# peterrum/deal-and-ceed-on-gpu

Measured on AMD Instinct MI355X. Metric: BP5 DoFs/sec per CG iter (p=4, ~1e8 DoFs) + % HBM roofline at 1/2/4/8 GPUs, higher is better.
Workload: dtype f64

## Files before the change

### deal-and-ceed-on-gpu_amd/_lib.py

```python
import ctypes as C
import os
import re
import subprocess

import numpy as np

_HERE = os.path.dirname(os.path.abspath(__file__))
_ROOT = os.path.dirname(_HERE)
_LIB = None

QUAD_GAUSS, QUAD_GLL, QUAD_GAUSS_OVER = 0, 1, 2
COEF_ONE, COEF_STEP64 = 0, 1
CG_PLAIN, CG_MERGED = 0, 1
GEOM_MERGED6, GEOM_AFFINE, GEOM_TRILINEAR = 0, 1, 2
OP_POISSON, OP_HELMHOLTZ, OP_MASS = 0, 1, 2
UNIQUE_ID_BYTES = 128
MAX_COMPONENTS = 8


class BP5Error(RuntimeError):
    def __init__(self, status, detail):
        super().__init__(f"bp5 status {status}: {detail}")
        self.status = status

# ... 123 lines not shown
        "bp5_mf_compute_merged_metric": (i32, [vp, vp]),
        "bp5_mf_metric_to_reference_layout": (i32, [vp, vp, vp]),
        "bp5_mf_set_geometry_mode": (i32, [vp, i32]),
        "bp5_mf_get_data": (i32, [vp, i32, C.POINTER(MFData)]),
        "bp5_apply": (i32, [vp, vp, vp, vp, i32]),
        "bp5_apply_cells": (i32, [vp, vp, vp, vp, u32, u32]),
        "bp5_apply_components": (i32, [vp, vp, i32, sz, vp, vp, i32]),
        "bp5_copy_constrained": (i32, [vp, vp, vp]),
        "bp5_set_constrained": (i32, [vp, f64, vp]),
        "bp5_mf_set_apply_variant": (i32, [vp, i32]),
        "bp5_mf_get_apply_variant": (i32, [vp, C.POINTER(C.c_int)]),
        "bp5_mf_set_block_workgroups": (i32, [vp, i32]),
        "bp5_mf_set_streaming": (i32, [vp, i32]),
        "bp5_mf_set_tuning": (i32, [vp, i32, i32]),
        "bp5_mf_get_tuning": (i32, [vp, i32, C.POINTER(C.c_int)]),
        "bp5_mf_wait_value_available": (i32, [vp, C.POINTER(C.c_int)]),
        "bp5_mf_block_plan_info": (i32, [vp, C.POINTER(C.c_uint32), C.POINTER(C.c_uint32), C.POINTER(C.c_int)]),
        "bp5_assemble_rhs": (i32, [vp, vp]),
        "bp5_compute_diagonal": (i32, [vp, vp, vp, i32]),
        "bp5_l2_norm_solution": (i32, [vp, vp, C.POINTER(f64)]),
        "bp5_vec_fill": (i32, [vp, vp, f64, sz]),
        "bp5_vec_axpy": (i32, [vp, vp, f64, vp, sz]),
        "bp5_vec_equ": (i32, [vp, vp, f64, vp, sz]),
        "bp5_vec_sadd": (i32, [vp, vp, f64, f64, vp, sz]),
        "bp5_vec_dot": (i32, [vp, vp, vp, sz, C.POINTER(f64)]),
        "bp5_vec_l2_norm": (i32, [vp, vp, C.c_size_t, C.POINTER(C.c_double)]),
        "bp5_vec_all_zero": (i32, [vp, vp, C.c_size_t, C.POINTER(C.c_int)]),
        "bp5_comm_unique_id": (i32, [vp]),
        "bp5_comm_create": (i32, [vp, i32, i32, C.POINTER(vp)]),
        "bp5_comm_destroy": (i32, [vp]),
# ... 105 lines not shown
```

### deal-and-ceed-on-gpu_amd/csrc/bp5_device.hip

```cpp
#include "bp5_device.hpp"


extern "C" int bp5_device_count(int *count)
{
  if (!count) return fail(BP5_ERR_INVALID, "null argument");
  int c = 0;
  hipError_t e = hipGetDeviceCount(&c);
  if (e != hipSuccess) { *count = 0; return fail(BP5_ERR_NO_DEVICE, hipGetErrorString(e)); }
  *count = c;
  return BP5_OK;
}
extern "C" int bp5_vec_alloc(size_t n, double **out)
{
  if (!out) return fail(BP5_ERR_INVALID, "null argument");
  HIP_TRY(hipMalloc((void **)out, std::max<size_t>(n, 1) * sizeof(double)));
  HIP_TRY(hipMemset(*out, 0, std::max<size_t>(n, 1) * sizeof(double)));
  HIP_TRY(hipStreamSynchronize(nullptr));
  return BP5_OK;
}
extern "C" int bp5_vec_free(double *v) { HIP_TRY(hipFree(v)); return BP5_OK; }
extern "C" int bp5_copy_h2d(void *dst, const void *src, size_t bytes) { HIP_TRY(hipMemcpy(dst, src, bytes, hipMemcpyHostToDevice)); return BP5_OK; }
extern "C" int bp5_copy_d2h(void *dst, const void *src, size_t bytes) { HIP_TRY(hipMemcpy(dst, src, bytes, hipMemcpyDeviceToHost)); return BP5_OK; }

static void tuning_from_environment(bp5_mf *mf);
// ... 139 lines not shown
  HIP_TRY(hipHostMalloc((void **)&mf->h_st, ST_COUNT * sizeof(int)));
  HIP_TRY(hipEventCreate(&mf->ev_solve[0]));
  HIP_TRY(hipEventCreate(&mf->ev_solve[1]));
  guard.m = nullptr;
  *out = mf;
  return BP5_OK;
}

extern "C" int bp5_mf_destroy(bp5_mf *mf)
{
  if (!mf) return BP5_OK;
  hipSetDevice(mf->device);
  hipStreamSynchronize(mf->stream);
  void *ptrs[] = {mf->d_constrained_bits, mf->d_l2g, mf->d_constrained, mf->d_send_idx, mf->d_coords, mf->d_tab, mf->d_tab_gauss, mf->d_l2g_padded,
                  mf->d_constraint_mask, mf->d_inv_jac, mf->d_JxW, mf->d_qpoints, mf->d_sendbuf, mf->d_recvbuf, mf->d_partials,
                  mf->d_sc, mf->d_scalar, mf->d_st, mf->ws_base, mf->d_stamps, mf->d_evec, mf->d_scalar_plane, mf->d_gcell, mf->d_vertices, mf->d_hang_mask, mf->d_hang_I, mf->d_send_dirichlet, mf->d_signal, mf->ws_z, mf->wsc_base, mf->wsz_base, mf->wsn_base, mf->hc_base, mf->d_hc_off};
  for (void *p : ptrs) if (p) hipFree(p);
  if (mf->h_sc) hipHostFree(mf->h_sc);
  if (mf->h_st) hipHostFree(mf->h_st);
  for (hipEvent_t e : mf->ev_pool) hipEventDestroy(e);
  for (hipEvent_t e : mf->phase.ev) hipEventDestroy(e);
  for (hipEvent_t e : mf->ev_solve) if (e) hipEventDestroy(e);
  for (hipEvent_t e : mf->ev_halo) if (e) hipEventDestroy(e);
  for (hipEvent_t e : mf->ev_done) if (e) hipEventDestroy(e);
  if (mf->h_done) hipHostFree(mf->h_done);
  if (mf->comm_stream) { hipStreamSynchronize(mf->comm_stream); hipStreamDestroy(mf->comm_stream); }
  for (auto &kv : mf->march_plans) { hipFree(kv.second.team_off); hipFree(kv.second.entries); }
  for (auto &kv : mf->plans) {
    auto &q = kv.second;
    void *pp[] = {q.off, q.dofs, q.sh_dof, q.sh_off, q.sh_slot, q.pos, q.cell_round, q.team_rounds, q.partial, q.cell_off, q.pass_cell, q.pass_off, q.run_off, q.runs, q.gidx, q.packed, q.lattice, q.cell_pos, q.cr_start, q.cr_dof0, q.cr_soff, q.cr_slots, q.cr_tile};
    for (void *x : pp) if (x) hipFree(x);
// ... 833 lines not shown
      const uint32_t grid = combine_grid(mf, owned_tiles, fuse->n_cols);
      if (ct.n_shared >= (8u << 20)) hipLaunchKernelGGL((combine_runs_kernel<false, true, true>), dim3(grid + cr.ghost_blocks), dim3(256), 0, stream, cr, dp->partial, dst);
      else hipLaunchKernelGGL((combine_runs_kernel<false, true, false>), dim3(grid + cr.ghost_blocks), dim3(256), 0, stream, cr, dp->partial, dst);
      KERNEL_CHECK();
      fuse->n_cols += grid;
      mf->signal_target += cr.ghost_blocks;
      return BP5_OK;
    }
    if (tile1 <= cr.tile0) return BP5_OK;
    const dim3 cgt(tile1 - cr.tile0);
    if (fuse && window != COMBINE_GHOST) {
      cr.cg_p = fuse->p; cr.cg_r = fuse->r; cr.dot_partials = mf->d_partials; cr.dot_col0 = fuse->n_cols;
      cr.n_owned = mf->n_owned; cr.n_tiles = cgt.x; cr.cg_state = mf->d_st;
      if (fuse->n_cols + 1024u + 8u > (uint32_t)PARTIAL_STRIDE) return fail(BP5_ERR_UNSUPPORTED, "no partial-sum columns left for the combine pass");
      const uint32_t grid = combine_grid(mf, cgt.x, fuse->n_cols);
      if (ct.n_shared >= (8u << 20)) hipLaunchKernelGGL((combine_runs_kernel<false, true, true>), dim3(grid), dim3(256), 0, stream, cr, dp->partial, dst);
      else hipLaunchKernelGGL((combine_runs_kernel<false, true, false>), dim3(grid), dim3(256), 0, stream, cr, dp->partial, dst);
      KERNEL_CHECK();
      fuse->n_cols += grid;
      return BP5_OK;
    }
    const bool pairs = ct.n_shared >= (8u << 20) && window != COMBINE_GHOST;
    if (set && pairs) hipLaunchKernelGGL((combine_runs_kernel<false, false, true>), cgt, dim3(256), 0, stream, cr, dp->partial, dst);
    else if (set) hipLaunchKernelGGL((combine_runs_kernel<false, false, false>), cgt, dim3(256), 0, stream, cr, dp->partial, dst);
    else if (pairs) hipLaunchKernelGGL((combine_runs_kernel<true, false, true>), cgt, dim3(256), 0, stream, cr, dp->partial, dst);
    else hipLaunchKernelGGL((combine_runs_kernel<true, false, false>), cgt, dim3(256), 0, stream, cr, dp->partial, dst);
    KERNEL_CHECK();
    return BP5_OK;
  }
  if (set) hipLaunchKernelGGL(combine_kernel<false>, cg, dim3(256), 0, stream, dp->sh_dof, dp->sh_off, dp->sh_slot, dp->partial, dst, dp->n_shared);
  else hipLaunchKernelGGL(combine_kernel<true>, cg, dim3(256), 0, stream, dp->sh_dof, dp->sh_off, dp->sh_slot, dp->partial, dst, dp->n_shared);
  KERNEL_CHECK();
  return BP5_OK;
}
// ... 546 lines not shown
static void tuning_from_environment(bp5_mf *mf)
{
  mf->tune[BP5_TUNE_LATTICE_INDICES] = env_int("BP5_LATTICE_INDICES", 1) != 0;
  mf->tune[BP5_TUNE_EARLY_GATHER] = env_int("BP5_EARLY_GATHER", 1) != 0;
  mf->tune[BP5_TUNE_COMBINE_SIGNAL] = env_int("BP5_COMBINE_SIGNAL", 0) == 1;
  { const char *e = getenv("BP5_BOUNDARY_FIRST"); mf->tune[BP5_TUNE_BOUNDARY_FIRST] = !(e && !strcmp(e, "launches")); }
  mf->tune[BP5_TUNE_FOLD_SMALL] = env_int("BP5_FOLD_SMALL", 1) != 0;
  { const int u = env_int("BP5_UPDATE_UNROLL", 1); mf->tune[BP5_TUNE_UPDATE_UNROLL] = (u == 2 || u == 4) ? u : 1; }
  mf->tune[BP5_TUNE_UPDATE_FLAT] = env_int("BP5_UPDATE_FLAT", 1) != 0;
  { const int v = env_int("BP5_UPDATE_NT", -1); mf->tune[BP5_TUNE_UPDATE_NT] = v < 0 ? -1 : v != 0; }
  { const int v = env_int("BP5_COMBINE_WG_PER_CU", 16); mf->tune[BP5_TUNE_COMBINE_WG_PER_CU] = (v >= 0 && v <= 32) ? v : 16; }
  mf->tune[BP5_TUNE_INTERIOR_STORES] = env_int("BP5_INTERIOR_STORES", 1) != 0;
  mf->tune[BP5_TUNE_GHOST_COMBINE_ON_COMM] = env_int("BP5_GHOST_COMBINE_ON_COMM", 0) != 0;
  mf->tune[BP5_TUNE_FACE_CARRY] = env_int("BP5_FACE_CARRY", 1) != 0;
  { const int v = env_int("BP5_FUSED_UPDATE", -1); mf->tune[BP5_TUNE_FUSED_UPDATE] = (v >= -1 && v <= 1) ? v : -1; }
}
extern "C" int bp5_mf_set_tuning(bp5_mf *mf, int knob, int value)
{
  if (!mf || knob < 0 || knob >= BP5_TUNE_COUNT) return fail(BP5_ERR_INVALID, "unknown tuning knob");
  switch (knob) {
    case BP5_TUNE_UPDATE_UNROLL:
      if (value != 1 && value != 2 && value != 4) return fail(BP5_ERR_INVALID, "BP5_TUNE_UPDATE_UNROLL: 1, 2 or 4");
      break;
    case BP5_TUNE_UPDATE_NT:
      if (value < -1 || value > 1) return fail(BP5_ERR_INVALID, "BP5_TUNE_UPDATE_NT: -1, 0 or 1");
      break;
    case BP5_TUNE_FUSED_UPDATE:
      if (value < -1 || value > 1) return fail(BP5_ERR_INVALID, "BP5_TUNE_FUSED_UPDATE: -1, 0 or 1");
      break;
    case BP5_TUNE_COMBINE_WG_PER_CU:
// ... 460 lines not shown
    while ((size_t)used + 4 > mf->ev_pool.size()) { hipEvent_t e; HIP_TRY(hipEventCreate(&e)); mf->ev_pool.push_back(e); }
    HIP_TRY(hipEventRecord(mf->ev_pool[used + k], mf->stream));
    return BP5_OK;
  }
};

struct SolveState {
  ApplyProfile prof;
  int exchange = EXCHANGE_NONE;
  bool two_parts = false;
  bool gather_in_flight = false;
  bool dst_prezeroed = false, copies_dirichlet = false;
  int upd_mode = 0;
  double *upd_x = nullptr;
  const double *upd_diag = nullptr;
  bool phase_on = false;
  int phase_it = 0;
  uint8_t phase_recorded[bp5_mf::PhaseProfile::MAX_ITERS] = {};
};

static int phase_mark(bp5_mf *mf, SolveState &ss, int k)
{
  if (!ss.phase_on || ss.phase_it >= bp5_mf::PhaseProfile::MAX_ITERS) return BP5_OK;
  HIP_TRY(hipEventRecord(mf->phase.ev[(size_t)ss.phase_it * bp5_mf::PhaseProfile::MARKS + k], mf->stream));
  ss.phase_recorded[ss.phase_it] |= (uint8_t)(1u << k);
  return BP5_OK;
}

static int fused_unsplit(bp5_mf *mf, SolveState &ss, ApplyCall &call, const double *coef, const double *src, double *dst)
{
// ... 117 lines not shown
    BP5_TRY(prof.mark(3));
    if (prof.on) prof.used += 4;
    BP5_TRY(bp5_halo_zero_ghosts(mf, src));
    return bp5_copy_constrained(mf, src, dst);
  }
  const bool owner_scatter = variant_overwrites(mf, effective_variant(mf, 0, mf->n_cells));
  BP5_TRY(prof.mark(0));
  if (zero && !owner_scatter) {
    if (!ss.dst_prezeroed) HIP_TRY(hipMemsetAsync(dst, 0, mf->n_local() * sizeof(double), mf->stream));
    zero = false;
    call.dst_known_zero = true;
  }
  BP5_TRY(prof.mark(1));
  if (prof.on) call.mark_event = mf->ev_pool[prof.used + 2];
  FuseState fuse;
  if (fusing) { fuse.p = src; fuse.r = fuse_r; fuse.upd_mode = ss.upd_mode; fuse.upd_x = ss.upd_x; fuse.upd_diag = ss.upd_diag; call.fuse = &fuse; }
  call.overwrite = zero;
  BP5_TRY(launch_apply(mf, call, coef, src, dst));
  if (fusing) *n_cols = fuse.n_cols;
  if (!call.mark_recorded) BP5_TRY(prof.mark(2));
  BP5_TRY(prof.mark(3));
  if (prof.on) prof.used += 4;
  if (fusing) return BP5_OK;
  if (ss.copies_dirichlet) return BP5_OK;
  return bp5_copy_constrained(mf, src, dst);
}

static int poll_state(bp5_mf *mf)
{
  HIP_TRY(hipMemcpyAsync(mf->h_st, mf->d_st, ST_COUNT * sizeof(int), hipMemcpyDeviceToHost, mf->stream));
  HIP_TRY(hipMemcpyAsync(mf->h_sc, mf->d_sc, SC_COUNT * sizeof(double), hipMemcpyDeviceToHost, mf->stream));
  HIP_TRY(hipStreamSynchronize(mf->stream));
  return BP5_OK;
}

static int solve_begin(bp5_mf *mf, const bp5_cg_params *prm, const ApplyProfile &prof)
{
  hipStream_t s = mf->stream;
  if (prof.on) {
    const size_t want = 4 * (size_t)std::min(prm->max_iter, ApplyProfile::MAX_PROFILED);
// ... 278 lines not shown
#undef BP5_UPR
  };
  const bool early_gather_enabled = mf->tune[BP5_TUNE_EARLY_GATHER] != 0;
  const bool early_gather = fused && dist_solve && early_gather_enabled;
  auto gather_under_update = [&](int mode) -> int {
    BP5_TRY(halo_streams(mf));
    const uint32_t ns = mf->send_off.back();
    if (ns) {
      const dim3 gr((ns + 255) / 256), bl(256);
      if (mode == 0) hipLaunchKernelGGL(cgm_pack_updated_kernel<0>, gr, bl, 0, s, mf->d_send_idx, ns, d, g, h, diag, mf->d_sc, mf->d_st, mf->d_sendbuf);
      else hipLaunchKernelGGL(cgm_pack_updated_kernel<1>, gr, bl, 0, s, mf->d_send_idx, ns, d, g, h, diag, mf->d_sc, mf->d_st, mf->d_sendbuf);
      KERNEL_CHECK();
    }
    return gather_exchange(mf, d, true);
  };
  int it = 1;
  for (; it <= prm->max_iter; ++it) {
    const int mode = it == 1 ? 0 : it % 2 == 0 ? 1 : 2;
    BP5_TRY(phase_mark(mf, ss, 0));
    if (early_gather) { BP5_TRY(gather_under_update(mode)); ss.gather_in_flight = true; }
    if (mode != 0) {
      if (n_first) launch_update_rest(mode); else launch_update(mode);
    }
    ss.upd_mode = n_first ? mode : 0; ss.upd_x = x; ss.upd_diag = diag;
    KERNEL_CHECK();
    BP5_TRY(phase_mark(mf, ss, 1));
    const bool one_launch = fused && !mf->comm;
    if (fused) {
      uint32_t n_cols = 0;
      BP5_TRY(vmult(d, h, g, &n_cols));
      BP5_TRY(phase_mark(mf, ss, 4));
      if (one_launch) hipLaunchKernelGGL(cgm_finalize4_kernel<true>, dim3(1), dim3(FIN4_THREADS), 0, s, mf->d_partials, (int)n_cols, mf->d_sc, mf->d_st);
      else hipLaunchKernelGGL(cgm_finalize4_kernel<false>, dim3(1), dim3(FIN4_THREADS), 0, s, mf->d_partials, (int)n_cols, mf->d_sc, mf->d_st);
    } else {
      BP5_TRY(vmult(d, h, nullptr, nullptr));
      BP5_TRY(phase_mark(mf, ss, 4));
      hipLaunchKernelGGL(cgm_dots_kernel, dim3(grid2), dim3(VB), 0, s, d, g, h, diag, n, mf->d_st, mf->d_partials,
                         fold_small ? (const uint32_t *)mf->d_constrained_bits : (const uint32_t *)nullptr);
      hipLaunchKernelGGL(finalize_kernel<7>, dim3(7), dim3(VB), 0, s, mf->d_partials, grid2, mf->d_sc + SC_R0, mf->d_st);
    }
    KERNEL_CHECK();
    BP5_TRY(phase_mark(mf, ss, 5));
    if (!one_launch) {
      BP5_TRY(bp5_comm_allreduce_sum(mf, mf->d_sc + SC_R0, 7));
      BP5_TRY(phase_mark(mf, ss, 6));
      hipLaunchKernelGGL(cgm_control_kernel, dim3(1), dim3(1), 0, s, mf->d_sc, mf->d_st);
      KERNEL_CHECK();
// ... 1038 lines not shown
```

### deal-and-ceed-on-gpu_amd/csrc/bp5_device.hpp

```cpp
#pragma once
#include "bp5_internal.hpp"
#include "bp5_kernels.hpp"

#include <hip/hip_runtime.h>
#include <rccl/rccl.h>

#include <algorithm>
#include <cmath>
#include <cstdio>
#include <cstdlib>
#include <cstring>
#include <map>
#include <memory>
#include <tuple>
#include <vector>

using namespace bp5;

#define HIP_TRY(expr)                                                                                              \
  do {                                                                                                             \
    hipError_t e_ = (expr);                                                                                        \
    if (e_ != hipSuccess)                                                                                          \
      return fail(e_ == hipErrorNoDevice || e_ == hipErrorInvalidDevice ? BP5_ERR_NO_DEVICE : BP5_ERR_HIP,         \
                  std::string(#expr) + ": " + hipGetErrorString(e_));                                              \
// ... 53 lines not shown
  uint32_t pad = 0;
  std::vector<int> neighbors;
  std::vector<uint32_t> send_off, recv_off;
  double *d_sendbuf = nullptr, *d_recvbuf = nullptr;
  uint8_t *d_send_dirichlet = nullptr;
  bp5_comm *comm = nullptr;
  hipStream_t comm_stream = nullptr;
  hipEvent_t ev_halo[4] = {nullptr, nullptr, nullptr, nullptr};
  int overlap = 2;
  bool overlap_now = false;
  bool cg_fusion = true;
  unsigned long long *d_signal = nullptr;
  uint64_t signal_target = 0;
  int wait_value_ok = -1;
  int can_wait_value = -1;
  int tune[BP5_TUNE_COUNT] = {1, 1, 0, 1, 1, 1, 1, -1, 16, 1, 0, 1, -1};
  bool cell_interiors_first = false;
  double *d_partials = nullptr, *d_sc = nullptr, *d_scalar = nullptr;
  int *d_st = nullptr;
  double *ws_g = nullptr, *ws_d = nullptr, *ws_h = nullptr, *d_evec = nullptr;
  char *ws_base = nullptr;
  double *ws_z = nullptr;
  double *wsc_base = nullptr;
  size_t wsc_cap = 0;
  double *wsz_base = nullptr;
  size_t wsz_cap = 0;
  double *wsn_base = nullptr;
  size_t wsn_cap = 0;
  double *hc_base = nullptr;
  size_t hc_cap = 0;
  uint32_t *d_hc_off = nullptr;
// ... 37 lines not shown
  std::vector<uint32_t> h_block_off;
  struct DevMarch { uint32_t *team_off = nullptr, *entries = nullptr; uint32_t n_teams = 0; };
  std::map<int, DevMarch> march_plans;
  std::map<int, DevPlan> plans;
  size_t n_local() const { return (size_t)n_owned + n_ghost; }
  bool has_neighbors() const { return comm && !neighbors.empty(); }
};

struct FuseState {
  const double *p = nullptr, *r = nullptr;
  uint32_t n_cols = 0;
  bool ghosts_zeroed = false;
  int upd_mode = 0;
  double *upd_x = nullptr;
  const double *upd_diag = nullptr;
};
enum VariantFamily { VARIANT_PENCIL, VARIANT_TEAM, VARIANT_MARCH, VARIANT_BLOCK, VARIANT_BLOCK_SIBLING, VARIANT_HANGING_PENCIL, VARIANT_OTHER };
struct VariantInfo {
  VariantFamily family;
  bool atomic_scatter;
  bool shared_by_atomics;
  bool csr_combine;
  bool overwrites;
};
constexpr VariantInfo decode_variant(int v)
{
  const int b = v % 100;
  const VariantFamily f = b <= 6 ? VARIANT_PENCIL : b >= 10 && b <= 14 ? VARIANT_TEAM : b == 56 ? VARIANT_BLOCK : b >= 48 && b <= 63 ? VARIANT_BLOCK_SIBLING
                        : b >= 70 && b <= 72 ? VARIANT_MARCH : b == 90 ? VARIANT_HANGING_PENCIL : VARIANT_OTHER;
  return {f, v >= 100, b == 54 || b == 55, b == 48, v < 100 && (f == VARIANT_TEAM || f == VARIANT_BLOCK || f == VARIANT_BLOCK_SIBLING)};
// ... 829 lines not shown
```

### deal-and-ceed-on-gpu_amd/csrc/bp5_kernels.hpp

```cpp
#pragma once
#include <hip/hip_runtime.h>
#include <stdint.h>
#include <type_traits>

namespace bp5 {

template <int n>
struct ShapeArg {
  double N[n * n];
  double D[n * n];
};

enum : int {
  BLK_AFFINE = 1024, BLK_SINGLE = 2048, BLK_STAMPS = 4096, BLK_SEQ = 8192, BLK_RUNS = 16384, BLK_NTM = 32768, BLK_UPD = 131072, BLK_PACK = 262144,
  BLK_STAGE = 524288, BLK_FUSE = 1048576, BLK_HANG = 2097152, BLK_LDSADD = 4194304, BLK_HELM = 8388608, BLK_LATT = 16777216,
  BLK_ROLL = 67108864, BLK_CARRY = 268435456,
  BLK_F32M = 536870912,
  BLK_MASS = 1073741824,
  BLK_DEFAULT = BLK_SINGLE | BLK_SEQ | BLK_RUNS | BLK_PACK
};
enum : int {
  PEN_INTERIOR_STORES = 32,
  PEN_NT_LOADS = 256,
  PEN_FULL_OCCUPANCY = 512
// ... 3494 lines not shown
  for (uint32_t j = b + 1; j < e; ++j) s += partial[sh_slot[j]];
  const uint32_t g = sh_dof[i];
  if (ADD) dst[g] += s; else dst[g] = s;
}

struct CombineRuns {
  const uint32_t *start, *dof0, *soff, *slots, *tile_run;
  uint32_t n_shared;
  uint32_t tile0, dof_lo, dof_hi;
  const double *cg_p, *cg_r;
  double *dot_partials;
  uint32_t dot_col0, n_owned, n_tiles;
  const int *cg_state;
  uint32_t ghost_blocks, ghost_tile0;
  unsigned long long *signal;
};
constexpr int COMBINE_TILE = 512;
template <bool ADD, bool DOTS = false, bool PAIR = true>
__global__ void __launch_bounds__(256) combine_runs_kernel(CombineRuns cr, const double *partial, double *dst)
{
  __shared__ uint32_t s_start[COMBINE_TILE + 2], s_dof0[COMBINE_TILE + 1], s_soff[COMBINE_TILE + 2];
  __shared__ double s_red[4][4];
  double ds[4] = {0.0, 0.0, 0.0, 0.0};
  const bool ghost_job = DOTS && blockIdx.x < cr.ghost_blocks;
  const uint32_t bid = blockIdx.x - (DOTS ? cr.ghost_blocks : 0u), nblk = gridDim.x - (DOTS ? cr.ghost_blocks : 0u);
  auto ghost_rows_done = [&](bool stores_pending) {
    if (stores_pending) __syncthreads();
    if (threadIdx.x == 0) {
      if (stores_pending) __builtin_amdgcn_fence(__ATOMIC_RELEASE, "agent");
      __hip_atomic_fetch_add(cr.signal, 1ull, __ATOMIC_RELAXED, __HIP_MEMORY_SCOPE_AGENT);
    }
  };
  if constexpr (DOTS) {
    if (cr.cg_state[0]) {
      if (ghost_job) ghost_rows_done(false);
      return;
    }
  }
  const uint32_t dof_lo = ghost_job ? cr.n_owned : cr.dof_lo, dof_hi = ghost_job ? 0xffffffffu : cr.dof_hi;
  auto finish = [&](uint32_t g, bool dirichlet, double s) {
    if (g < dof_lo || g >= dof_hi) return;
    if (ghost_job) { dst[g] = s; return; }
    if constexpr (DOTS) {
      double vi = s;
      if (dirichlet) {
        vi = cr.cg_p[g];
        if (g < cr.n_owned) ds[0] += vi * (vi - s);
      }
      dst[g] = vi;
      if (g < cr.n_owned) {
// ... 183 lines not shown
    }
  }
  if constexpr (DOTS) {
    if (ghost_job) { ghost_rows_done(true); return; }
    const int lane = threadIdx.x & 63, wave = threadIdx.x >> 6;
#pragma unroll
    for (int k = 0; k < 4; ++k) {
      double v = ds[k];
#pragma unroll
      for (int off = 32; off > 0; off >>= 1) v += __shfl_down(v, off, 64);
      if (lane == 0) s_red[k][wave] = v;
    }
    __syncthreads();
    if (threadIdx.x < 7) {
      const int t = threadIdx.x, k = t < 4 ? t : (t == 4 ? 2 : t == 5 ? 1 : 3);
      cr.dot_partials[t * PARTIAL_STRIDE + cr.dot_col0 + bid] = (s_red[k][0] + s_red[k][1]) + (s_red[k][2] + s_red[k][3]);
    }
  }
}

static __global__ void __launch_bounds__(256) zero_indexed_kernel(const uint32_t *idx, uint32_t n, double *dst)
{
  const uint32_t i = blockIdx.x * 256u + threadIdx.x;
  if (i < n) dst[idx[i]] = 0.0;
}

static __global__ void copy_constrained_kernel(const uint32_t *cdofs, uint32_t n, const double *src, double *dst)
{
  const uint32_t i = blockIdx.x * blockDim.x + threadIdx.x;
  if (i < n) { const uint32_t c = cdofs[i]; dst[c] = src[c]; }
}
// ... 384 lines not shown
template <int MODE, int U = 2, bool ZV = false, bool NTX = false>
__global__ void __launch_bounds__(VB) cgm_update_kernel(double *p, double *r, typename std::conditional<ZV, double, const double>::type *v, double *x,
                                                       const double *diag, size_t n, const double *sc, const int *st)
{
  const bool done = st[ST_DONE];
  if (done && !st[ST_PENDING]) return;
  cgm_update_body<MODE, U, ZV, NTX>(p, r, v, x, diag, n, sc, st, done);
}
template <int MODE, int U, bool NTX>
__global__ void __launch_bounds__(VB) cgm_update_rest_kernel(double *p, double *r, const double *v, double *x, const double *diag, size_t first, size_t n,
                                                            const double *sc, const int *st)
{
  if (st[ST_DONE]) return;
  cgm_update_body<MODE, U, false, NTX>(p + first, r + first, v + first, x + first, diag ? diag + first : nullptr, n, sc, st, false);
}
#ifndef BP5_UPD_UNROLL
#define BP5_UPD_UNROLL 3
#endif
template <int MODE>
__device__ __forceinline__ void block_update_run(const BlockPlan &bp, uint32_t lo, uint32_t hi, int t)
{
  static_assert(MODE == 1 || MODE == 2, "the first iteration's p comes from cgm_init_kernel");
  constexpr int U = BP5_UPD_UNROLL;
  constexpr uint32_t TRIP = 2u * 256u;
  const double *sc = bp.upd_sc;
  const double alpha = sc[SC_ALPHA], beta = sc[SC_BETA];
  const double aob = MODE == 2 ? sc[SC_ALPHA_OLD] / sc[SC_BETA_OLD] : 0.0;
  double *const p = bp.upd_p, *const r = bp.upd_r, *const x = bp.upd_x;
  const double *const v = bp.upd_v, *const diag = bp.upd_diag;
  for (uint32_t base = lo + 2u * (uint32_t)t; base < hi; base += TRIP * U) {
    bp5_d2u pv[U], rv[U], vv[U], xv[U];
#pragma unroll
    for (int u = 0; u < U; ++u) {
      const uint32_t i = base + (uint32_t)u * TRIP;
      pv[u] = rv[u] = vv[u] = xv[u] = bp5_d2u{0.0, 0.0};
      if (i + 1 < hi) {
        pv[u] = __builtin_nontemporal_load(reinterpret_cast<const bp5_d2u *>(p + i));
        rv[u] = __builtin_nontemporal_load(reinterpret_cast<const bp5_d2u *>(r + i));
        vv[u] = __builtin_nontemporal_load(reinterpret_cast<const bp5_d2u *>(v + i));
        if (MODE == 2) xv[u] = __builtin_nontemporal_load(reinterpret_cast<const bp5_d2u *>(x + i));
      } else if (i < hi) {
        pv[u].x = __builtin_nontemporal_load(p + i); rv[u].x = __builtin_nontemporal_load(r + i); vv[u].x = __builtin_nontemporal_load(v + i);
        if (MODE == 2) xv[u].x = __builtin_nontemporal_load(x + i);
      }
    }
#pragma unroll
    for (int u = 0; u < U; ++u) {
      const uint32_t i = base + (uint32_t)u * TRIP;
      if (i >= hi) continue;
      const bool pair = i + 1 < hi;
      double p0 = pv[u].x, p1 = pv[u].y, r0 = rv[u].x, r1 = rv[u].y, x0 = xv[u].x, x1 = xv[u].y;
      cgm_update_one<MODE>(p0, r0, vv[u].x, x0, diag ? diag[i] : 1.0, false, false, alpha, beta, aob);
      if (pair) {
        cgm_update_one<MODE>(p1, r1, vv[u].y, x1, diag ? diag[i + 1] : 1.0, false, false, alpha, beta, aob);
        *reinterpret_cast<bp5_d2u *>(p + i) = bp5_d2u{p0, p1};
        *reinterpret_cast<bp5_d2u *>(r + i) = bp5_d2u{r0, r1};
        if (MODE == 2) __builtin_nontemporal_store(bp5_d2u{x0, x1}, reinterpret_cast<bp5_d2u *>(x + i));
      } else {
        p[i] = p0; r[i] = r0;
        if (MODE == 2) __builtin_nontemporal_store(x0, x + i);
      }
    }
  }
}
template <int MODE>
__global__ void __launch_bounds__(256) cgm_pack_updated_kernel(const uint32_t *idx, uint32_t n, const double *p, const double *r, const double *v,
                                                             const double *diag, const double *sc, const int *st, double *buf)
{
  const uint32_t i = blockIdx.x * 256u + threadIdx.x;
  if (i >= n) return;
  const uint32_t g = idx[i];
  double pi = p[g];
  if (!st[ST_DONE]) {
    double ri = r[g], xi = 0.0;
    const double vi = MODE != 0 ? v[g] : 0.0;
    cgm_update_one<MODE>(pi, ri, vi, xi, diag ? diag[g] : 1.0, false, false, sc[SC_ALPHA], sc[SC_BETA], 0.0);
  }
  buf[i] = pi;
// ... 69 lines not shown
  if (lane == 0) red[wave] = s;
  __syncthreads();
  double *out = sc + SC_R0;
  if (threadIdx.x < 4) {
    const int r = threadIdx.x;
    const double t = (red[4 * r] + red[4 * r + 1]) + (red[4 * r + 2] + red[4 * r + 3]);
    out[r] = t;
    if (r == 1) out[5] = t;
    if (r == 2) out[4] = t;
    if (r == 3) out[6] = t;
  }
  if constexpr (CONTROL) {
    __syncthreads();
    if (threadIdx.x == 0) cgm_control_step(sc, st);
  }
}

static __global__ void cgm_control_kernel(double *sc, int *st) { cgm_control_step(sc, st); }

static __global__ void __launch_bounds__(VB) cgm_init_kernel(const double *b, double *x, double *r, double *p, double *v, const double *diag, size_t n,
                                                     double *partials, bool zero_v)
{
  double acc[2] = {0.0, 0.0};
  const size_t stride = (size_t)gridDim.x * VB;
  for (size_t i = (size_t)blockIdx.x * VB + threadIdx.x; i < n; i += stride) {
    const double ri = -b[i], di = diag ? diag[i] : 1.0;
    x[i] = 0.0; r[i] = ri; p[i] = -(di * ri);
    if (zero_v) v[i] = 0.0;
    acc[0] += ri * ri;
  }
// ... 1119 lines not shown
```

### deal-and-ceed-on-gpu_amd/matrix_free.py

```python
import ctypes as C

import numpy as np

from . import _lib
from ._lib import BP5Error, CG_MERGED, CG_PLAIN, COEF_ONE, QUAD_GAUSS


def _torch():
    import torch
    return torch


def _ptr(t, n_min=0):
    torch = _torch()
    if t is None:
        return None
    if not (isinstance(t, torch.Tensor) and t.is_cuda and t.dtype == torch.float64 and t.is_contiguous()):
        raise BP5Error(1, "expected a contiguous float64 CUDA tensor")
    if t.numel() < n_min:
        raise BP5Error(1, f"vector has {t.numel()} entries, need {n_min}")
    return C.c_void_p(t.data_ptr())


class Communicator:
# ... 120 lines not shown
            raise BP5Error(1, f"metric precision must be 'float64' or 'float32', not {precision!r}")
        _lib.check(_lib.lib().bp5_mf_set_metric_precision(self.handle, self.METRIC_PRECISION[precision]))

    def get_metric_precision(self):
        v = C.c_int()
        _lib.check(_lib.lib().bp5_mf_get_metric_precision(self.handle, C.byref(v)))
        return "float32" if v.value == 1 else "float64"

    def set_block_workgroups(self, n):
        _lib.check(_lib.lib().bp5_mf_set_block_workgroups(self.handle, int(n)))

    def set_streaming(self, policy):
        _lib.check(_lib.lib().bp5_mf_set_streaming(self.handle, int(policy)))

    TUNE = {"lattice_indices": 0, "early_gather": 1, "combine_signal": 2, "boundary_first": 3, "fold_small": 4, "update_unroll": 5,
            "update_flat": 6, "update_nt": 7, "combine_wg_per_cu": 8, "interior_stores": 9, "ghost_combine_on_comm": 10, "face_carry": 11, "fused_update": 12}

    def set_tuning(self, knob, value):
        _lib.check(_lib.lib().bp5_mf_set_tuning(self.handle, int(self.TUNE.get(knob, knob)), int(value)))

    def get_tuning(self, knob):
        v = C.c_int()
        _lib.check(_lib.lib().bp5_mf_get_tuning(self.handle, int(self.TUNE.get(knob, knob)), C.byref(v)))
        return v.value

    def wait_value_available(self):
        v = C.c_int()
        _lib.check(_lib.lib().bp5_mf_wait_value_available(self.handle, C.byref(v)))
        return bool(v.value)

    def block_plan_info(self):
        nb, mr, pk = C.c_uint32(), C.c_uint32(), C.c_int()
        _lib.check(_lib.lib().bp5_mf_block_plan_info(self.handle, C.byref(nb), C.byref(mr), C.byref(pk)))
        return nb.value, mr.value, bool(pk.value)

    def block_plan_lattice(self):
        n = C.c_uint32()
        _lib.check(_lib.lib().bp5_mf_block_plan_lattice(self.handle, C.byref(n)))
        return n.value
# ... 955 lines not shown
```

### include/bp5.h

```cpp
#ifndef BP5_H
#define BP5_H

#include <stddef.h>
#include <stdint.h>

#ifdef __cplusplus
extern "C" {
#endif

enum {
  BP5_OK = 0,
  BP5_ERR_INVALID = 1,
  BP5_ERR_HIP = 2,
  BP5_ERR_NO_DEVICE = 3,
  BP5_ERR_RCCL = 4,
  BP5_ERR_UNSUPPORTED = 5,
  BP5_ERR_BREAKDOWN = 6,
  BP5_ERR_NO_CONVERGENCE = 7
};
const char *bp5_strerror(int status);
const char *bp5_last_error(void);

enum { BP5_QUAD_GAUSS = 0,
       BP5_QUAD_GLL = 1,
// ... 113 lines not shown
int bp5_apply(bp5_mf *mf, const double *coef, const double *src, double *dst, int zero_dst);
int bp5_apply_cells(bp5_mf *mf, const double *coef, const double *src, double *dst, uint32_t cell_begin,
                    uint32_t cell_end);
int bp5_copy_constrained(bp5_mf *mf, const double *src, double *dst);
int bp5_set_constrained(bp5_mf *mf, double value, double *dst);

#define BP5_MAX_COMPONENTS 8
int bp5_apply_components(bp5_mf *mf, const double *coef, int n_components, size_t ld, const double *src, double *dst, int zero_dst);

int bp5_mf_set_apply_variant(bp5_mf *mf, int variant);
int bp5_mf_set_block_workgroups(bp5_mf *mf, int max_workgroups);
int bp5_mf_set_streaming(bp5_mf *mf, int policy);
enum { BP5_TUNE_LATTICE_INDICES = 0, BP5_TUNE_EARLY_GATHER = 1, BP5_TUNE_COMBINE_SIGNAL = 2, BP5_TUNE_BOUNDARY_FIRST = 3,
       BP5_TUNE_FOLD_SMALL = 4, BP5_TUNE_UPDATE_UNROLL = 5, BP5_TUNE_UPDATE_FLAT = 6, BP5_TUNE_UPDATE_NT = 7, BP5_TUNE_COMBINE_WG_PER_CU = 8,
       BP5_TUNE_INTERIOR_STORES = 9, BP5_TUNE_GHOST_COMBINE_ON_COMM = 10, BP5_TUNE_FACE_CARRY = 11, BP5_TUNE_FUSED_UPDATE = 12,
       BP5_TUNE_COUNT = 13 };
int bp5_mf_set_tuning(bp5_mf *mf, int knob, int value);
int bp5_mf_get_tuning(const bp5_mf *mf, int knob, int *value);
int bp5_mf_wait_value_available(bp5_mf *mf, int *available);
int bp5_mf_block_plan_info(bp5_mf *mf, uint32_t *n_blocks, uint32_t *max_runs, int *packed_indices);
int bp5_mf_block_plan_lattice(bp5_mf *mf, uint32_t *n_lattice_blocks);
int bp5_mf_block_plan_carry(bp5_mf *mf, uint32_t *n_faces, uint32_t *n_shared, uint32_t *n_shared_last_launch);
int bp5_mf_get_apply_variant(bp5_mf *mf, int *effective);

int bp5_compute_diagonal(bp5_mf *mf, const double *coef, double *diag, int invert);

int bp5_assemble_rhs(bp5_mf *mf, double *b);
int bp5_l2_norm_solution(bp5_mf *mf, const double *u, double *result_host);

int bp5_vec_fill(bp5_mf *mf, double *v, double value, size_t n);
int bp5_vec_axpy(bp5_mf *mf, double *y, double a, const double *x, size_t n);
int bp5_vec_equ(bp5_mf *mf, double *y, double a, const double *x, size_t n);
int bp5_vec_sadd(bp5_mf *mf, double *y, double s, double a, const double *x, size_t n);
// ... 178 lines not shown
```

Baseline: 30.23 billion.

## Fold CG scalar finalize into last combine workgroup via atomic counter

In the single-GPU fused CG path, the last workgroup of the combine kernel (found with an atomic ticket counter) now reduces the dot-product partials and runs the CG control step. This replaces the separate cgm_finalize4 launch and the launch gap it adds to every iteration. It also splits the block-update unroll factor by mode (4 for mode 1, 3 for mode 2). The cost is atomic-store and fence ordering in every combine block, plus a serial reduction tail in one workgroup.

```diff
diff --git a/deal-and-ceed-on-gpu_amd/_lib.py b/deal-and-ceed-on-gpu_amd/_lib.py
--- a/deal-and-ceed-on-gpu_amd/_lib.py
+++ b/deal-and-ceed-on-gpu_amd/_lib.py
@@ -161,6 +161,7 @@
         "bp5_mf_set_streaming": (i32, [vp, i32]),
         "bp5_mf_set_tuning": (i32, [vp, i32, i32]),
         "bp5_mf_get_tuning": (i32, [vp, i32, C.POINTER(C.c_int)]),
+        "bp5_mf_last_cg_scalars": (i32, [vp, C.POINTER(C.c_double), C.POINTER(C.c_double)]),
         "bp5_mf_wait_value_available": (i32, [vp, C.POINTER(C.c_int)]),
         "bp5_mf_block_plan_info": (i32, [vp, C.POINTER(C.c_uint32), C.POINTER(C.c_uint32), C.POINTER(C.c_int)]),
         "bp5_assemble_rhs": (i32, [vp, vp]),
diff --git a/deal-and-ceed-on-gpu_amd/csrc/bp5_device.hip b/deal-and-ceed-on-gpu_amd/csrc/bp5_device.hip
--- a/deal-and-ceed-on-gpu_amd/csrc/bp5_device.hip
+++ b/deal-and-ceed-on-gpu_amd/csrc/bp5_device.hip
@@ -177,7 +177,7 @@
   hipStreamSynchronize(mf->stream);
   void *ptrs[] = {mf->d_constrained_bits, mf->d_l2g, mf->d_constrained, mf->d_send_idx, mf->d_coords, mf->d_tab, mf->d_tab_gauss, mf->d_l2g_padded,
                   mf->d_constraint_mask, mf->d_inv_jac, mf->d_JxW, mf->d_qpoints, mf->d_sendbuf, mf->d_recvbuf, mf->d_partials,
-                  mf->d_sc, mf->d_scalar, mf->d_st, mf->ws_base, mf->d_stamps, mf->d_evec, mf->d_scalar_plane, mf->d_gcell, mf->d_vertices, mf->d_hang_mask, mf->d_hang_I, mf->d_send_dirichlet, mf->d_signal, mf->ws_z, mf->wsc_base, mf->wsz_base, mf->wsn_base, mf->hc_base, mf->d_hc_off};
+                  mf->d_sc, mf->d_scalar, mf->d_st, mf->ws_base, mf->d_stamps, mf->d_evec, mf->d_scalar_plane, mf->d_gcell, mf->d_vertices, mf->d_hang_mask, mf->d_hang_I, mf->d_send_dirichlet, mf->d_signal, mf->d_fold_count, mf->ws_z, mf->wsc_base, mf->wsz_base, mf->wsn_base, mf->hc_base, mf->d_hc_off};
   for (void *p : ptrs) if (p) hipFree(p);
   if (mf->h_sc) hipHostFree(mf->h_sc);
   if (mf->h_st) hipHostFree(mf->h_st);
@@ -1041,10 +1041,17 @@
       cr.n_owned = mf->n_owned; cr.n_tiles = cgt.x; cr.cg_state = mf->d_st;
       if (fuse->n_cols + 1024u + 8u > (uint32_t)PARTIAL_STRIDE) return fail(BP5_ERR_UNSUPPORTED, "no partial-sum columns left for the combine pass");
       const uint32_t grid = combine_grid(mf, cgt.x, fuse->n_cols);
-      if (ct.n_shared >= (8u << 20)) hipLaunchKernelGGL((combine_runs_kernel<false, true, true>), dim3(grid), dim3(256), 0, stream, cr, dp->partial, dst);
+      const bool pairs = ct.n_shared >= (8u << 20);
+      const bool fold = fuse->fold_step && window == COMBINE_ALL && !on_comm_stream && mf->d_fold_count;
+      if (fold) {
+        cr.fold_sc = mf->d_sc; cr.fold_st = mf->d_st; cr.fold_count = mf->d_fold_count; cr.fold_cols = fuse->n_cols + grid;
+        if (pairs) hipLaunchKernelGGL((combine_runs_kernel<false, true, true, true>), dim3(grid), dim3(256), 0, stream, cr, dp->partial, dst);
+        else hipLaunchKernelGGL((combine_runs_kernel<false, true, false, true>), dim3(grid), dim3(256), 0, stream, cr, dp->partial, dst);
+      } else if (pairs) hipLaunchKernelGGL((combine_runs_kernel<false, true, true>), dim3(grid), dim3(256), 0, stream, cr, dp->partial, dst);
       else hipLaunchKernelGGL((combine_runs_kernel<false, true, false>), dim3(grid), dim3(256), 0, stream, cr, dp->partial, dst);
       KERNEL_CHECK();
       fuse->n_cols += grid;
+      fuse->step_folded = fold;
       return BP5_OK;
     }
     const bool pairs = ct.n_shared >= (8u << 20) && window != COMBINE_GHOST;
@@ -1621,6 +1628,7 @@
   mf->tune[BP5_TUNE_GHOST_COMBINE_ON_COMM] = env_int("BP5_GHOST_COMBINE_ON_COMM", 0) != 0;
   mf->tune[BP5_TUNE_FACE_CARRY] = env_int("BP5_FACE_CARRY", 1) != 0;
   { const int v = env_int("BP5_FUSED_UPDATE", -1); mf->tune[BP5_TUNE_FUSED_UPDATE] = (v >= -1 && v <= 1) ? v : -1; }
+  mf->tune[BP5_TUNE_FOLD_STEP] = env_int("BP5_FOLD_STEP", 1) != 0;
 }
 extern "C" int bp5_mf_set_tuning(bp5_mf *mf, int knob, int value)
 {
@@ -2111,6 +2119,7 @@
   int upd_mode = 0;
   double *upd_x = nullptr;
   const double *upd_diag = nullptr;
+  bool fold_step = false, step_folded = false;
   bool phase_on = false;
   int phase_it = 0;
   uint8_t phase_recorded[bp5_mf::PhaseProfile::MAX_ITERS] = {};
@@ -2258,16 +2267,24 @@
   BP5_TRY(prof.mark(1));
   if (prof.on) call.mark_event = mf->ev_pool[prof.used + 2];
   FuseState fuse;
-  if (fusing) { fuse.p = src; fuse.r = fuse_r; fuse.upd_mode = ss.upd_mode; fuse.upd_x = ss.upd_x; fuse.upd_diag = ss.upd_diag; call.fuse = &fuse; }
+  if (fusing) { fuse.p = src; fuse.r = fuse_r; fuse.upd_mode = ss.upd_mode; fuse.upd_x = ss.upd_x; fuse.upd_diag = ss.upd_diag; fuse.fold_step = ss.fold_step; call.fuse = &fuse; }
   call.overwrite = zero;
+  ss.step_folded = false;
   BP5_TRY(launch_apply(mf, call, coef, src, dst));
-  if (fusing) *n_cols = fuse.n_cols;
+  if (fusing) { *n_cols = fuse.n_cols; ss.step_folded = fuse.step_folded; }
   if (!call.mark_recorded) BP5_TRY(prof.mark(2));
   BP5_TRY(prof.mark(3));
   if (prof.on) prof.used += 4;
   if (fusing) return BP5_OK;
   if (ss.copies_dirichlet) return BP5_OK;
   return bp5_copy_constrained(mf, src, dst);
+}
+
+extern "C" int bp5_mf_last_cg_scalars(const bp5_mf *mf, double *alpha, double *beta)
+{
+  if (!mf || !alpha || !beta) return fail(BP5_ERR_INVALID, "bp5_mf_last_cg_scalars: null argument");
+  *alpha = mf->h_sc[SC_ALPHA]; *beta = mf->h_sc[SC_BETA];
+  return BP5_OK;
 }
 
 static int poll_state(bp5_mf *mf)
@@ -2576,6 +2593,11 @@
     }
     return gather_exchange(mf, d, true);
   };
+  const bool fold_step = fused && !user && !mf->comm && mf->tune[BP5_TUNE_FOLD_STEP] != 0;
+  if (fold_step) {
+    if (!mf->d_fold_count) HIP_TRY(hipMalloc((void **)&mf->d_fold_count, sizeof(uint32_t)));
+    HIP_TRY(hipMemsetAsync(mf->d_fold_count, 0, sizeof(uint32_t), s));
+  }
   int it = 1;
   for (; it <= prm->max_iter; ++it) {
     const int mode = it == 1 ? 0 : it % 2 == 0 ? 1 : 2;
@@ -2590,9 +2612,11 @@
     const bool one_launch = fused && !mf->comm;
     if (fused) {
       uint32_t n_cols = 0;
+      ss.fold_step = one_launch && fold_step;
       BP5_TRY(vmult(d, h, g, &n_cols));
       BP5_TRY(phase_mark(mf, ss, 4));
-      if (one_launch) hipLaunchKernelGGL(cgm_finalize4_kernel<true>, dim3(1), dim3(FIN4_THREADS), 0, s, mf->d_partials, (int)n_cols, mf->d_sc, mf->d_st);
+      if (one_launch && ss.step_folded) {}
+      else if (one_launch) hipLaunchKernelGGL(cgm_finalize4_kernel<true>, dim3(1), dim3(FIN4_THREADS), 0, s, mf->d_partials, (int)n_cols, mf->d_sc, mf->d_st);
       else hipLaunchKernelGGL(cgm_finalize4_kernel<false>, dim3(1), dim3(FIN4_THREADS), 0, s, mf->d_partials, (int)n_cols, mf->d_sc, mf->d_st);
     } else {
       BP5_TRY(vmult(d, h, nullptr, nullptr));
diff --git a/deal-and-ceed-on-gpu_amd/csrc/bp5_device.hpp b/deal-and-ceed-on-gpu_amd/csrc/bp5_device.hpp
--- a/deal-and-ceed-on-gpu_amd/csrc/bp5_device.hpp
+++ b/deal-and-ceed-on-gpu_amd/csrc/bp5_device.hpp
@@ -91,7 +91,8 @@
   uint64_t signal_target = 0;
   int wait_value_ok = -1;
   int can_wait_value = -1;
-  int tune[BP5_TUNE_COUNT] = {1, 1, 0, 1, 1, 1, 1, -1, 16, 1, 0, 1, -1};
+  int tune[BP5_TUNE_COUNT] = {1, 1, 0, 1, 1, 1, 1, -1, 16, 1, 0, 1, -1, 1};
+  uint32_t *d_fold_count = nullptr;
   bool cell_interiors_first = false;
   double *d_partials = nullptr, *d_sc = nullptr, *d_scalar = nullptr;
   int *d_st = nullptr;
@@ -159,6 +160,7 @@
   int upd_mode = 0;
   double *upd_x = nullptr;
   const double *upd_diag = nullptr;
+  bool fold_step = false, step_folded = false;
 };
 enum VariantFamily { VARIANT_PENCIL, VARIANT_TEAM, VARIANT_MARCH, VARIANT_BLOCK, VARIANT_BLOCK_SIBLING, VARIANT_HANGING_PENCIL, VARIANT_OTHER };
 struct VariantInfo {
diff --git a/deal-and-ceed-on-gpu_amd/csrc/bp5_kernels.hpp b/deal-and-ceed-on-gpu_amd/csrc/bp5_kernels.hpp
--- a/deal-and-ceed-on-gpu_amd/csrc/bp5_kernels.hpp
+++ b/deal-and-ceed-on-gpu_amd/csrc/bp5_kernels.hpp
@@ -3532,11 +3532,18 @@
   const int *cg_state;
   uint32_t ghost_blocks, ghost_tile0;
   unsigned long long *signal;
+  double *fold_sc;
+  int *fold_st;
+  uint32_t *fold_count;
+  uint32_t fold_cols;
 };
+__device__ __forceinline__ void cgm_finalize4_rows256(const double *partials, int nblk, double *sc, int *st, double (*red)[4]);
+__device__ __forceinline__ void cgm_control_step(double *sc, int *st);
 constexpr int COMBINE_TILE = 512;
-template <bool ADD, bool DOTS = false, bool PAIR = true>
+template <bool ADD, bool DOTS = false, bool PAIR = true, bool FOLD = false>
 __global__ void __launch_bounds__(256) combine_runs_kernel(CombineRuns cr, const double *partial, double *dst)
 {
+  static_assert(!FOLD || (DOTS && !ADD), "the folded scalar step belongs to the fused solver's combine launch");
   __shared__ uint32_t s_start[COMBINE_TILE + 2], s_dof0[COMBINE_TILE + 1], s_soff[COMBINE_TILE + 2];
   __shared__ double s_red[4][4];
   double ds[4] = {0.0, 0.0, 0.0, 0.0};
@@ -3552,6 +3559,7 @@
   if constexpr (DOTS) {
     if (cr.cg_state[0]) {
       if (ghost_job) ghost_rows_done(false);
+      if (FOLD && blockIdx.x == 0 && threadIdx.x == 0) cgm_control_step(cr.fold_sc, cr.fold_st);
       return;
     }
   }
@@ -3765,7 +3773,24 @@
     __syncthreads();
     if (threadIdx.x < 7) {
       const int t = threadIdx.x, k = t < 4 ? t : (t == 4 ? 2 : t == 5 ? 1 : 3);
-      cr.dot_partials[t * PARTIAL_STRIDE + cr.dot_col0 + bid] = (s_red[k][0] + s_red[k][1]) + (s_red[k][2] + s_red[k][3]);
+      const double col = (s_red[k][0] + s_red[k][1]) + (s_red[k][2] + s_red[k][3]);
+      if constexpr (FOLD) __hip_atomic_store(cr.dot_partials + t * PARTIAL_STRIDE + cr.dot_col0 + bid, col, __ATOMIC_RELAXED, __HIP_MEMORY_SCOPE_AGENT);
+      else cr.dot_partials[t * PARTIAL_STRIDE + cr.dot_col0 + bid] = col;
+    }
+    if constexpr (FOLD) {
+      asm volatile("s_waitcnt vmcnt(0)" ::: "memory");
+      if (threadIdx.x == 0) {
+        const bool last = __hip_atomic_fetch_add(cr.fold_count, 1u, __ATOMIC_RELAXED, __HIP_MEMORY_SCOPE_AGENT) == nblk - 1u;
+        if (last) {
+          __builtin_amdgcn_fence(__ATOMIC_ACQUIRE, "agent");
+          asm volatile("s_waitcnt vmcnt(0)" ::: "memory");
+        }
+        s_start[0] = last ? 1u : 0u;
+      }
+      __syncthreads();
+      if (!s_start[0]) return;
+      cgm_finalize4_rows256(cr.dot_partials, (int)cr.fold_cols, cr.fold_sc, cr.fold_st, s_red);
+      if (threadIdx.x == 0) __hip_atomic_store(cr.fold_count, 0u, __ATOMIC_RELAXED, __HIP_MEMORY_SCOPE_AGENT);
     }
   }
 }
@@ -4180,54 +4205,61 @@
   if (st[ST_DONE]) return;
   cgm_update_body<MODE, U, false, NTX>(p + first, r + first, v + first, x + first, diag ? diag + first : nullptr, n, sc, st, false);
 }
-#ifndef BP5_UPD_UNROLL
-#define BP5_UPD_UNROLL 3
+#ifndef BP5_UPD_UNROLL1
+#define BP5_UPD_UNROLL1 4
 #endif
+#ifndef BP5_UPD_UNROLL2
+#define BP5_UPD_UNROLL2 3
+#endif
+struct BlockUpdateScalars { double alpha, beta, aob; };
+template <int MODE, int U>
+__device__ __forceinline__ void block_update_trip(const BlockPlan &bp, const BlockUpdateScalars &k, uint32_t base, uint32_t hi)
+{
+  constexpr uint32_t TRIP = 2u * 256u;
+  double *const p = bp.upd_p, *const r = bp.upd_r, *const x = bp.upd_x;
+  const double *const v = bp.upd_v, *const diag = bp.upd_diag;
+  bp5_d2u pv[U], rv[U], vv[U], xv[U];
+#pragma unroll
+  for (int u = 0; u < U; ++u) {
+    const uint32_t i = base + (uint32_t)u * TRIP;
+    pv[u] = rv[u] = vv[u] = xv[u] = bp5_d2u{0.0, 0.0};
+    if (i + 1 < hi) {
+      pv[u] = __builtin_nontemporal_load(reinterpret_cast<const bp5_d2u *>(p + i));
+      rv[u] = __builtin_nontemporal_load(reinterpret_cast<const bp5_d2u *>(r + i));
+      vv[u] = __builtin_nontemporal_load(reinterpret_cast<const bp5_d2u *>(v + i));
+      if (MODE == 2) xv[u] = __builtin_nontemporal_load(reinterpret_cast<const bp5_d2u *>(x + i));
+    } else if (i < hi) {
+      pv[u].x = __builtin_nontemporal_load(p + i); rv[u].x = __builtin_nontemporal_load(r + i); vv[u].x = __builtin_nontemporal_load(v + i);
+      if (MODE == 2) xv[u].x = __builtin_nontemporal_load(x + i);
+    }
+  }
+#pragma unroll
+  for (int u = 0; u < U; ++u) {
+    const uint32_t i = base + (uint32_t)u * TRIP;
+    if (i >= hi) continue;
+    const bool pair = i + 1 < hi;
+    double p0 = pv[u].x, p1 = pv[u].y, r0 = rv[u].x, r1 = rv[u].y, x0 = xv[u].x, x1 = xv[u].y;
+    cgm_update_one<MODE>(p0, r0, vv[u].x, x0, diag ? diag[i] : 1.0, false, false, k.alpha, k.beta, k.aob);
+    if (pair) {
+      cgm_update_one<MODE>(p1, r1, vv[u].y, x1, diag ? diag[i + 1] : 1.0, false, false, k.alpha, k.beta, k.aob);
+      *reinterpret_cast<bp5_d2u *>(p + i) = bp5_d2u{p0, p1};
+      *reinterpret_cast<bp5_d2u *>(r + i) = bp5_d2u{r0, r1};
+      if (MODE == 2) __builtin_nontemporal_store(bp5_d2u{x0, x1}, reinterpret_cast<bp5_d2u *>(x + i));
+    } else {
+      p[i] = p0; r[i] = r0;
+      if (MODE == 2) __builtin_nontemporal_store(x0, x + i);
+    }
+  }
+}
 template <int MODE>
 __device__ __forceinline__ void block_update_run(const BlockPlan &bp, uint32_t lo, uint32_t hi, int t)
 {
   static_assert(MODE == 1 || MODE == 2, "the first iteration's p comes from cgm_init_kernel");
-  constexpr int U = BP5_UPD_UNROLL;
+  constexpr int U = MODE == 1 ? BP5_UPD_UNROLL1 : BP5_UPD_UNROLL2;
   constexpr uint32_t TRIP = 2u * 256u;
   const double *sc = bp.upd_sc;
-  const double alpha = sc[SC_ALPHA], beta = sc[SC_BETA];
-  const double aob = MODE == 2 ? sc[SC_ALPHA_OLD] / sc[SC_BETA_OLD] : 0.0;
-  double *const p = bp.upd_p, *const r = bp.upd_r, *const x = bp.upd_x;
-  const double *const v = bp.upd_v, *const diag = bp.upd_diag;
-  for (uint32_t base = lo + 2u * (uint32_t)t; base < hi; base += TRIP * U) {
-    bp5_d2u pv[U], rv[U], vv[U], xv[U];
-#pragma unroll
-    for (int u = 0; u < U; ++u) {
-      const uint32_t i = base + (uint32_t)u * TRIP;
-      pv[u] = rv[u] = vv[u] = xv[u] = bp5_d2u{0.0, 0.0};
-      if (i + 1 < hi) {
-        pv[u] = __builtin_nontemporal_load(reinterpret_cast<const bp5_d2u *>(p + i));
-        rv[u] = __builtin_nontemporal_load(reinterpret_cast<const bp5_d2u *>(r + i));
-        vv[u] = __builtin_nontemporal_load(reinterpret_cast<const bp5_d2u *>(v + i));
-        if (MODE == 2) xv[u] = __builtin_nontemporal_load(reinterpret_cast<const bp5_d2u *>(x + i));
-      } else if (i < hi) {
-        pv[u].x = __builtin_nontemporal_load(p + i); rv[u].x = __builtin_nontemporal_load(r + i); vv[u].x = __builtin_nontemporal_load(v + i);
-        if (MODE == 2) xv[u].x = __builtin_nontemporal_load(x + i);
-      }
-    }
-#pragma unroll
-    for (int u = 0; u < U; ++u) {
-      const uint32_t i = base + (uint32_t)u * TRIP;
-      if (i >= hi) continue;
-      const bool pair = i + 1 < hi;
-      double p0 = pv[u].x, p1 = pv[u].y, r0 = rv[u].x, r1 = rv[u].y, x0 = xv[u].x, x1 = xv[u].y;
-      cgm_update_one<MODE>(p0, r0, vv[u].x, x0, diag ? diag[i] : 1.0, false, false, alpha, beta, aob);
-      if (pair) {
-        cgm_update_one<MODE>(p1, r1, vv[u].y, x1, diag ? diag[i + 1] : 1.0, false, false, alpha, beta, aob);
-        *reinterpret_cast<bp5_d2u *>(p + i) = bp5_d2u{p0, p1};
-        *reinterpret_cast<bp5_d2u *>(r + i) = bp5_d2u{r0, r1};
-        if (MODE == 2) __builtin_nontemporal_store(bp5_d2u{x0, x1}, reinterpret_cast<bp5_d2u *>(x + i));
-      } else {
-        p[i] = p0; r[i] = r0;
-        if (MODE == 2) __builtin_nontemporal_store(x0, x + i);
-      }
-    }
-  }
+  const BlockUpdateScalars k{sc[SC_ALPHA], sc[SC_BETA], MODE == 2 ? sc[SC_ALPHA_OLD] / sc[SC_BETA_OLD] : 0.0};
+  for (uint32_t base = lo + 2u * (uint32_t)t; base < hi; base += TRIP * U) block_update_trip<MODE, U>(bp, k, base, hi);
 }
 template <int MODE>
 __global__ void __launch_bounds__(256) cgm_pack_updated_kernel(const uint32_t *idx, uint32_t n, const double *p, const double *r, const double *v,
@@ -4327,6 +4359,40 @@
     __syncthreads();
     if (threadIdx.x == 0) cgm_control_step(sc, st);
   }
+}
+
+__device__ __forceinline__ void cgm_finalize4_rows256(const double *partials, int nblk, double *sc, int *st, double (*red)[4])
+{
+  const int l = threadIdx.x, wave = l >> 6, lane = l & 63;
+  double s[4];
+#pragma unroll
+  for (int k = 0; k < 4; ++k) {
+    const double *row = partials + k * PARTIAL_STRIDE;
+    double s0 = 0.0, s1 = 0.0, s2 = 0.0, s3 = 0.0;
+    for (int i = l; i < nblk; i += 1024) {
+      const double a0 = row[i], a1 = i + 256 < nblk ? row[i + 256] : 0.0, a2 = i + 512 < nblk ? row[i + 512] : 0.0, a3 = i + 768 < nblk ? row[i + 768] : 0.0;
+      s0 += a0; s1 += a1; s2 += a2; s3 += a3;
+    }
+    s[k] = (s0 + s1) + (s2 + s3);
+  }
+#pragma unroll
+  for (int k = 0; k < 4; ++k) {
+    double v = s[k];
+#pragma unroll
+    for (int off = 32; off > 0; off >>= 1) v += __shfl_down(v, off, 64);
+    if (lane == 0) red[k][wave] = v;
+  }
+  __syncthreads();
+  double *out = sc + SC_R0;
+  if (l < 4) {
+    const double t = (red[l][0] + red[l][1]) + (red[l][2] + red[l][3]);
+    out[l] = t;
+    if (l == 1) out[5] = t;
+    if (l == 2) out[4] = t;
+    if (l == 3) out[6] = t;
+  }
+  __syncthreads();
+  if (l == 0) cgm_control_step(sc, st);
 }
 
 static __global__ void cgm_control_kernel(double *sc, int *st) { cgm_control_step(sc, st); }
diff --git a/deal-and-ceed-on-gpu_amd/matrix_free.py b/deal-and-ceed-on-gpu_amd/matrix_free.py
--- a/deal-and-ceed-on-gpu_amd/matrix_free.py
+++ b/deal-and-ceed-on-gpu_amd/matrix_free.py
@@ -158,7 +158,7 @@
         _lib.check(_lib.lib().bp5_mf_set_streaming(self.handle, int(policy)))
 
     TUNE = {"lattice_indices": 0, "early_gather": 1, "combine_signal": 2, "boundary_first": 3, "fold_small": 4, "update_unroll": 5,
-            "update_flat": 6, "update_nt": 7, "combine_wg_per_cu": 8, "interior_stores": 9, "ghost_combine_on_comm": 10, "face_carry": 11, "fused_update": 12}
+            "update_flat": 6, "update_nt": 7, "combine_wg_per_cu": 8, "interior_stores": 9, "ghost_combine_on_comm": 10, "face_carry": 11, "fused_update": 12, "fold_step": 13}
 
     def set_tuning(self, knob, value):
         _lib.check(_lib.lib().bp5_mf_set_tuning(self.handle, int(self.TUNE.get(knob, knob)), int(value)))
@@ -167,6 +167,11 @@
         v = C.c_int()
         _lib.check(_lib.lib().bp5_mf_get_tuning(self.handle, int(self.TUNE.get(knob, knob)), C.byref(v)))
         return v.value
+
+    def last_cg_scalars(self):
+        a, b = C.c_double(), C.c_double()
+        _lib.check(_lib.lib().bp5_mf_last_cg_scalars(self.handle, C.byref(a), C.byref(b)))
+        return a.value, b.value
 
     def wait_value_available(self):
         v = C.c_int()
diff --git a/include/bp5.h b/include/bp5.h
--- a/include/bp5.h
+++ b/include/bp5.h
@@ -151,9 +151,10 @@
 enum { BP5_TUNE_LATTICE_INDICES = 0, BP5_TUNE_EARLY_GATHER = 1, BP5_TUNE_COMBINE_SIGNAL = 2, BP5_TUNE_BOUNDARY_FIRST = 3,
        BP5_TUNE_FOLD_SMALL = 4, BP5_TUNE_UPDATE_UNROLL = 5, BP5_TUNE_UPDATE_FLAT = 6, BP5_TUNE_UPDATE_NT = 7, BP5_TUNE_COMBINE_WG_PER_CU = 8,
        BP5_TUNE_INTERIOR_STORES = 9, BP5_TUNE_GHOST_COMBINE_ON_COMM = 10, BP5_TUNE_FACE_CARRY = 11, BP5_TUNE_FUSED_UPDATE = 12,
-       BP5_TUNE_COUNT = 13 };
+       BP5_TUNE_FOLD_STEP = 13, BP5_TUNE_COUNT = 14 };
 int bp5_mf_set_tuning(bp5_mf *mf, int knob, int value);
 int bp5_mf_get_tuning(const bp5_mf *mf, int knob, int *value);
+int bp5_mf_last_cg_scalars(const bp5_mf *mf, double *alpha, double *beta);
 int bp5_mf_wait_value_available(bp5_mf *mf, int *available);
 int bp5_mf_block_plan_info(bp5_mf *mf, uint32_t *n_blocks, uint32_t *max_runs, int *packed_indices);
 int bp5_mf_block_plan_lattice(bp5_mf *mf, uint32_t *n_lattice_blocks);
```

After: 29.87 billion. 1.2% lower.
